# Orkis-Research/Quaternion-Convolutional-Neural-Networks-for-End-to-End-Automatic-Speech-Recognition

Measured on AMD Instinct MI355X. Metric: quaternion-conv samples/sec (fwd+bwd+Adam of the full TIMIT QCNN, per-GPU batch 256), higher is better.
Workload: dtype bf16; 1 GPU; cfg3_qcnn_relu_dropout_b256_bf16; per_gpu_batch=256, global_batch=256, filters=32, padding=same, activation=relu, loss=ctc, parallelism=dp1, optimizer=adam(5e-4) + l2 term folded into the update, launch=eager

## Files before the change

### quaternion-convolutional-neural-networks-for-end-to-end-automatic-speech-recognition_amd/csrc/qk_common.h

```cpp
#pragma once

#include <hip/hip_runtime.h>
#include <stdint.h>
#include <stdio.h>
#include <stdlib.h>

#include "../../include/qk.h"

namespace qk {

constexpr unsigned kSignConv = 0x5390u;
constexpr unsigned kSignConj = 0x284Eu;

struct PostOp {
    int kind;
    int alpha_sel;
    int alpha_len;
    const float *alpha;
    float drop_scale;
    unsigned drop_thr;
    unsigned drop_seed;
    const unsigned *seed_dev;
};

struct GemmGeom {
    int M;
    int batch;
    int osp[3];
    int isp[3];
    int Q;
    int J;
    int Qp, Jp;
    int ks[3];
    int taps;
    int pa[3], pb[3], pc[3], pd[3];
    long long in_sn, in_ss[3], in_sc;
    long long out_sn, out_ss, out_sc;
    unsigned sign_tbl;
    int relu;
    int has_bias;
    int has_mask;
    int ablate;
    unsigned b_rep;
    unsigned long long *dbg_ts;
    int w_swapped;
    int w_prepped;
    unsigned dv_mul[3], dv_shr[3];
    const void *ep_mask;
    PostOp post;
    int post_fwd;
    void *pre_out;
    float *dalpha;
    void *bits_out;
    const void *ep_bits;
    int b_wp, b_nlines, b_cshift, b_rev;
    int o0_major;
    unsigned b_in_bytes, b_w_bytes;
    int w_ch_major;
};

inline int pad32(int v) { return (v + 31) / 32 * 32; }
inline size_t band_image_bytes(int taps, int Qp, int Jp) { return (size_t)taps * Qp * 4 * Jp * 2 + 256; }

inline bool band_geom(const GemmGeom &g, int esize, GemmGeom *o)
{
    if (g.has_mask) return false;
    if (g.pd[0] != 1 || g.pd[1] != 1 || g.pd[2] != 1) return false;
    int ax = 2;
    while (ax > 0 && g.osp[ax] == 1 && g.isp[ax] == 1 && g.ks[ax] == 1) --ax;
    if (g.ks[ax] != 3 && g.ks[ax] != 5) return false;
    if (g.pa[ax] != 1 || (g.pb[ax] != 1 && g.pb[ax] != -1)) return false;
    *o = g;
    const int sh = 2 - ax;
    for (int i = 0; i < 3; ++i) {
        const int src = i - sh;
        o->osp[i] = src >= 0 ? g.osp[src] : 1; o->isp[i] = src >= 0 ? g.isp[src] : 1; o->ks[i] = src >= 0 ? g.ks[src] : 1;
        o->pa[i] = src >= 0 ? g.pa[src] : 1; o->pb[i] = src >= 0 ? g.pb[src] : 1; o->pc[i] = src >= 0 ? g.pc[src] : 0;
        o->in_ss[i] = src >= 0 ? g.in_ss[src] : 0;
    }
    const int k = o->ks[2];
    if (o->ks[0] * o->ks[1] > 32) return false;
    for (int i = 0; i < 2; ++i)
        if (o->pb[i] != 1 && o->pb[i] != -1) return false;
    o->b_rep = 0;
    for (int t0 = 0; t0 < o->ks[0]; ++t0) o->b_rep |= 1u << (t0 * o->ks[1]);
    o->b_wp = o->osp[2] + k - 1;
    if ((k - 1) * 12 > o->b_wp) return false;
    const long long lines = (long long)g.batch * o->osp[0] * o->osp[1];
    if (lines * o->b_wp >= (1ll << 31) - 512) return false;
    o->b_nlines = (int)lines;
    const int Qw = g.Qp ? g.Qp : g.Q, Jw = g.Jp ? g.Jp : g.J;
    const long long in_bytes = (long long)g.batch * g.in_sn * esize, w_bytes = (long long)band_image_bytes(g.taps, Qw, Jw);
    if (in_bytes >= 0xF0000000ll || w_bytes >= 0xF0000000ll) return false;
    o->b_in_bytes = (unsigned)in_bytes;
    o->b_w_bytes = (unsigned)w_bytes;
    o->b_rev = o->pb[2] < 0;
    o->b_cshift = o->b_rev ? o->pc[2] - (k - 1) : o->pc[2];
    if (o->post.alpha_sel >= 0) o->post.alpha_sel += sh;
    return true;
}


inline void fastdiv_of(unsigned d, unsigned *mul, unsigned *shr)
{
    if (d <= 1) { *mul = 0; *shr = 0; return; }
    unsigned lg = 0;
    while ((1ull << lg) < d) ++lg;
    const unsigned p = 31 + lg;
    *mul = (unsigned)(((1ull << p) + d - 1) / d);
    *shr = p - 32;
}
__device__ __forceinline__ int fastdiv(int n, unsigned mul, unsigned shr)
{
    const unsigned q = __umulhi((unsigned)n, mul) >> shr;
    const unsigned id = (unsigned)-(int)(mul == 0u);
    return (int)((q & ~id) | ((unsigned)n & id));
}

__device__ __forceinline__ unsigned outer_tap_mask(int q0, int q1, const GemmGeom &g)
{
    const int m0 = q0 * g.pb[0] + (g.pb[0] > 0 ? 0 : g.isp[0] - 1), m1q = q1 * g.pb[1] + (g.pb[1] > 0 ? 0 : g.isp[1] - 1);
    const int lo0 = max(0, -m0), hi0 = min(g.ks[0], g.isp[0] - m0);
    const int lo1 = max(0, -m1q), hi1 = min(g.ks[1], g.isp[1] - m1q);
    const unsigned m1 = ((hi1 >= 32 ? 0u : (1u << hi1)) - 1u) & ~((1u << lo1) - 1u);
    const int b0 = lo0 * g.ks[1], e0 = hi0 * g.ks[1];
    const unsigned r0 = ((e0 >= 32 ? 0u : (1u << e0)) - 1u) & ~((1u << b0) - 1u);
    return (lo0 >= hi0 || lo1 >= hi1) ? 0u : (m1 * g.b_rep) & r0;
}


struct WgradGeom {
    int M;
    int batch;
    int osp[3];
    int isp[3];
    int Cq, F;
    int ks[3];
    int taps;
    int pa[3], pb[3], pc[3];
    long long x_sn, x_ss[3], x_sc;
    long long dy_sn, dy_ss, dy_sc;
    unsigned sign_tbl;
    int has_mask;
    int want_dbias;
    int m_per_split;
    int n_splits;
    int ablate;
    int deterministic;
    unsigned x_bytes, dy_bytes;
    int b_wp, b_nlines, b_cshift;
    int w_ch_major;
    void *dym;
    unsigned fd_mul[4], fd_sh[4];
};

inline void make_fastdiv(unsigned d, unsigned *mul, unsigned *sh)
{
    unsigned s = 0;
    while ((1ull << s) < d) ++s;
    *mul = (unsigned)(((1ull << (31 + s)) + d - 1) / d);
    *sh = s;
}
__host__ __device__ __forceinline__ int fast_div(int n, unsigned mul, unsigned sh)
{
    return (int)(((unsigned long long)(unsigned)n * mul) >> (31 + sh));
}

struct bf16 { uint16_t x; };
typedef _Float16 f16;

__device__ __forceinline__ float to_f32(float v) { return v; }
__device__ __forceinline__ float to_f32(bf16 v) { return __uint_as_float(((uint32_t)v.x) << 16); }
__device__ __forceinline__ float to_f32(f16 v) { return (float)v; }

template <typename T> __device__ __forceinline__ T from_f32(float v);
template <> __device__ __forceinline__ float from_f32<float>(float v) { return v; }
template <> __device__ __forceinline__ bf16 from_f32<bf16>(float v)
{
    uint32_t u = __float_as_uint(v);
    bf16 r;
    if ((u & 0x7fffffffu) > 0x7f800000u) { r.x = (uint16_t)((u >> 16) | 0x40u); return r; }
    u += 0x7fffu + ((u >> 16) & 1u);
    r.x = (uint16_t)(u >> 16);
    return r;
}
template <> __device__ __forceinline__ f16 from_f32<f16>(float v) { return (f16)v; }

__device__ __forceinline__ void load4(const float *p, float (&o)[4])
{
    const float4 v = *reinterpret_cast<const float4 *>(p);
    o[0] = v.x; o[1] = v.y; o[2] = v.z; o[3] = v.w;
}
__device__ __forceinline__ void load4(const bf16 *p, float (&o)[4])
{
    const uint2 v = *reinterpret_cast<const uint2 *>(p);
    o[0] = __uint_as_float(v.x << 16); o[1] = __uint_as_float(v.x & 0xffff0000u);
    o[2] = __uint_as_float(v.y << 16); o[3] = __uint_as_float(v.y & 0xffff0000u);
}
__device__ __forceinline__ void load4(const f16 *p, float (&o)[4])
{
    typedef f16 h4 __attribute__((ext_vector_type(4)));
    const h4 v = *reinterpret_cast<const h4 *>(p);
    o[0] = (float)v[0]; o[1] = (float)v[1]; o[2] = (float)v[2]; o[3] = (float)v[3];
}

template <typename T>
__device__ __forceinline__ void prep_small16_write(const float *w, T *wq, long long idx, int Cq, int F, int transposed, int neg_ijk,
// ... 142 lines not shown
```

### quaternion-convolutional-neural-networks-for-end-to-end-automatic-speech-recognition_amd/csrc/qk_hgemm_bf16mfma.hip

```cpp
#include "qk_common.h"
#include "qk_postop.h"
#include <type_traits>

namespace qk {
namespace {

typedef __bf16 bf16x8 __attribute__((ext_vector_type(8)));
typedef _Float16 f16x8 __attribute__((ext_vector_type(8)));

__device__ __forceinline__ floatx16 mfma16(bf16, const uint4 &a, const uint4 &b, const floatx16 &c)
{
    return __builtin_amdgcn_mfma_f32_32x32x16_bf16(__builtin_bit_cast(bf16x8, a), __builtin_bit_cast(bf16x8, b), c, 0, 0, 0);
}
__device__ __forceinline__ floatx16 mfma16(f16, const uint4 &a, const uint4 &b, const floatx16 &c)
{
    return __builtin_amdgcn_mfma_f32_32x32x16_f16(__builtin_bit_cast(f16x8, a), __builtin_bit_cast(f16x8, b), c, 0, 0, 0);
}

typedef float f32x2 __attribute__((ext_vector_type(2)));
typedef __bf16 bf16x2 __attribute__((ext_vector_type(2)));
typedef _Float16 f16x2 __attribute__((ext_vector_type(2)));
__device__ __forceinline__ unsigned pack2(bf16, float a, float b)
{
    const f32x2 v = {a, b};
// ... 1083 lines not shown

inline bool point_geom(const GemmGeom &g, GemmGeom *o)
{
    if (g.has_mask || (g.Q != 32 && g.Q != 64) || g.J % 32 != 0) return false;
    if (g.post.kind != 0) {
        const bool epm = g.ep_mask || g.ep_bits;
        const bool fwd_relu = g.post_fwd && g.post.kind == 2 && !g.pre_out && !epm;
        if (!fwd_relu && (!epm || g.post_fwd || g.post.alpha_len > 256 || (g.taps == 1 && g.post.alpha_sel >= 0))) return false;
    }
    *o = g;
    if (g.taps == 1) {
        for (int i = 0; i < 3; ++i)
            if (g.pa[i] != 1 || g.pc[i] != 0 || g.isp[i] != g.osp[i]) return false;
        if (g.in_ss[1] != g.isp[2] * g.in_ss[2] || g.in_ss[0] != g.isp[1] * g.in_ss[1] || g.in_sn != g.isp[0] * g.in_ss[0]) return false;
        o->batch = g.M;
        o->in_sn = g.in_ss[2];
        for (int i = 0; i < 3; ++i) { o->osp[i] = o->isp[i] = 1; o->in_ss[i] = 0; }
    } else {
        if (g.ks[1] != 1 || g.ks[2] != 1 || g.isp[0] != 1 || g.ks[0] != g.osp[0]) return false;
        for (int i = 1; i < 3; ++i)
            if (g.pa[i] != 1 || g.pc[i] != 0 || g.isp[i] != g.osp[i]) return false;
        if (g.pc[0] != 0 || g.pa[0] != 1 || g.pb[0] != -1) return false;
    }
    if ((long long)o->batch * o->in_sn * 2 >= (1ll << 31) || (long long)g.M * g.out_ss >= (1ll << 31)) return false;
    return true;
}

template <typename T>
int run16_point(const T *in, const uint4 *wq, const float *bias, T *out, GemmGeom g, hipStream_t stream)
{
    const int S = g.osp[1] * g.osp[2], R = g.batch * S;
    fastdiv_of((unsigned)g.osp[2], &g.dv_mul[0], &g.dv_shr[0]);
    fastdiv_of((unsigned)g.osp[1], &g.dv_mul[1], &g.dv_shr[1]);
    fastdiv_of((unsigned)S, &g.dv_mul[2], &g.dv_shr[2]);
    const bool wide = g.J % 64 == 0;
    const int BM = wide ? 128 : 256, BF = wide ? 64 : 32;
    const int n_tiles = (R + BM - 1) / BM;
    const int n_units = g.ks[0] * (g.J / BF) * n_tiles;
    int blocks = device_cu_count();
    if (blocks > n_units) blocks = n_units;
    const unsigned in_bytes = (unsigned)((long long)g.batch * g.in_sn * 2);
    const unsigned out_bytes = (unsigned)((long long)g.M * g.out_ss * 2);
#define QK_GO(NKC, E, W) hipLaunchKernelGGL((k_hgemm16_point<T, NKC, E, W>), dim3(blocks), dim3(512), 0, stream, in, wq, bias, out, g, n_tiles, n_units, in_bytes, out_bytes)
    const int epm = g.ep_bits ? 2 : g.ep_mask ? 1 : 0;
#define QK_GO3(NKC, W) do { if (epm == 2) QK_GO(NKC, 2, W); else if (epm == 1) QK_GO(NKC, 1, W); else QK_GO(NKC, 0, W); } while (0)
    if (wide) { if (g.Q == 64) QK_GO3(2, 2); else QK_GO3(1, 2); }
    else      { if (g.Q == 64) QK_GO3(2, 1); else QK_GO3(1, 1); }
#undef QK_GO3
#undef QK_GO
    return hipGetLastError() == hipSuccess ? 1 : QK_ERR_LAUNCH;
}

template <typename T, int WM, int WN, int KIN, bool TRIM, bool PAD = false>
int run16_band(const T *in, const uint4 *wq, const T *zero_line, const float *bias, T *out, const GemmGeom &g,
               hipStream_t stream)
{
    constexpr int BM = WM * 32, BF = WN * 32, BMU = TRIM ? BM - (KIN - 1) : BM, NTHR = WM * WN * 64;
    const int n_mt = (int)(((long long)g.b_nlines * g.b_wp + BMU - 1) / BMU);
    dim3 grid((n_mt + 7) / 8 * 8, (PAD ? g.Jp : g.J) / BF, 1);
#define QK_GO(C, E, P) hipLaunchKernelGGL((k_hgemm16_band<T, WM, WN, KIN, C, TRIM, E, P, PAD>), grid, dim3(NTHR), (g.ablate & 64) ? 40960 : 0, stream, in, wq, zero_line, bias, out, g)
    const bool epm = g.ep_mask != nullptr, pf = g.post.kind != 0 && g.post_fwd != 0;
    if (g.sign_tbl != kSignConj) return QK_ERR_LAUNCH;
    if constexpr (!PAD && WM * WN == 4) {
        if (g.ep_bits) { QK_GO(true, 2, false); return hipGetLastError() == hipSuccess ? 1 : QK_ERR_LAUNCH; }
    }
    if (g.ep_bits || ((PAD || WM * WN != 4) && g.bits_out)) return QK_ERR_UNSUPPORTED;
    if (epm) QK_GO(true, 1, false); else if (pf) QK_GO(true, 0, true); else QK_GO(true, 0, false);
#undef QK_GO
    return hipGetLastError() == hipSuccess ? 1 : QK_ERR_LAUNCH;
}

template <typename T, int MT, int WM, int WN>
int run16(const T *in, const T *mask, const uint4 *wq, const T *zero_line, const float *bias, T *out,
          const GemmGeom &g_in, hipStream_t stream)
{
    constexpr int BM = WM * MT * 32, BF = WN * 32;
    const GemmGeom &g = g_in;
    const int n_mt = (g.M + BM - 1) / BM;
    dim3 grid((n_mt + 7) / 8 * 8, g.J / BF, 1);
    const bool m = g.has_mask != 0;
    if (g.sign_tbl != kSignConj) return QK_ERR_LAUNCH;
#define QK_GO(C, K) hipLaunchKernelGGL((k_hgemm16<T, MT, WM, WN, C, K>), grid, dim3(512), 0, stream, in, mask, wq, zero_line, bias, out, g)
    if (m) QK_GO(true, true); else QK_GO(true, false);
#undef QK_GO
    return hipGetLastError() == hipSuccess ? 1 : QK_ERR_LAUNCH;
}

template <typename T>
int go16(const void *in, const void *mask, const float *w, const float *bias, void *out, const GemmGeom &g_in,
         bool transposed, void *ws, size_t ws_bytes, hipStream_t stream)
{
    GemmGeom g = g_in;
    g.ablate = debug_ablate();
    { size_t nb = 0; g.dbg_ts = debug_buffer(&nb); if (nb < 64u * 65536u) g.dbg_ts = nullptr; }
    const bool neg_ijk = g.sign_tbl == kSignConv;
    g.sign_tbl = kSignConj;
    for (int i = 0; i < 3; ++i) fastdiv_of((unsigned)g.osp[2 - i], &g.dv_mul[i], &g.dv_shr[i]);
    T *wq = static_cast<T *>(ws);
    const int Cq = transposed ? g.J : g.Q, F = transposed ? g.Q : g.J;
    g.Qp = pad32(g.Q); g.Jp = pad32(g.J);
    const bool padded = g.Qp != g.Q || g.Jp != g.J;
    const bool bits = g.bits_out || g.ep_bits;
    if (bits && (padded || g.post.kind != 2)) return QK_ERR_UNSUPPORTED;
    GemmGeom bg;
    {
        Small16 sm;
        const size_t band_bytes = band_image_bytes(g.taps, g.Qp, g.Jp);
        if (!g.w_ch_major && small16_shape(g, &bg, &sm) && ws_bytes >= band_bytes + small16_region_bytes(sm)) {
            T *wqs = reinterpret_cast<T *>(static_cast<char *>(ws) + band_bytes);
            if (!g.w_prepped) {
// ... 127 lines not shown
```

### quaternion-convolutional-neural-networks-for-end-to-end-automatic-speech-recognition_amd/csrc/qk_hgemm_f32mfma.inc

```

namespace qk {
namespace {

struct RowPos { int n, o0, o1, o2; };

__device__ __forceinline__ RowPos decompose(int m, int M, const int (&osp)[3])
{
    RowPos r;
    if (m >= M) { r.n = -1; r.o0 = r.o1 = r.o2 = 0; return r; }
    int s = m;
    r.o2 = s % osp[2]; s /= osp[2];
    r.o1 = s % osp[1]; s /= osp[1];
    r.o0 = s % osp[0];
    r.n = s / osp[0];
    return r;
}

__device__ __forceinline__ bool axis_pos(int o, int t, int pa, int pb, int pc, int pd, int isp, int &i)
{
    const int num = o * pa + t * pb + pc;
    i = num;
    bool ok = num >= 0;
    if (pd != 1) {
        i = num / pd;
// ... 696 lines not shown
                    } else {
                        const int P = pt0 + row;
                        line = P / WP;
                        u = P - line * WP;
                    }
                    if (line >= g.b_nlines || u >= g.osp[2] || nvalid <= 0) continue;
                    float *dst = reinterpret_cast<float *>(out) + (size_t)(line * g.osp[2] + u) * (size_t)g.out_ss + ech;
                    if (nvalid >= 4) {
                        *reinterpret_cast<float4 *>(dst) = v;
                    } else {
                        dst[0] = v.x;
                        if (nvalid > 1) dst[1] = v.y;
                        if (nvalid > 2) dst[2] = v.z;
                    }
                }
            }
            return;
        }
    }
#pragma unroll
    for (int t = 0; t < NTILE; ++t) {
        if (!TP::valid(wave, t)) continue;
        const int jslot = TP::b_slot(t);
        const int j = j0 + cj[jslot];
        if (j >= g.J) continue;
        const int ch = cb[jslot] * g.J + j;
        const float bia = g.has_bias ? bias[ch] : 0.f;
        const int pt0 = p0 + TP::a_tile(wave, TP::a_slot(t)) * 32;
#pragma unroll
        for (int r = 0; r < 16; ++r) {
            int line, u;
            if (two_lines) {
                const int rr = rem0 + (pt0 - p0) + mfma32_row(r, lane);
                const bool second = rr >= WP;
                line = line0 + (second ? 1 : 0);
                u = second ? rr - WP : rr;
            } else {
                const int P = pt0 + mfma32_row(r, lane);
                line = P / WP;
                u = P - line * WP;
            }
            if (line >= g.b_nlines || u >= g.osp[2]) continue;
            float v = ((WIDE && w_sigma) ? -acc[t][r] : acc[t][r]) + bia;
            if (g.relu) v = v > 0.f ? v : 0.f;
            out[(line * g.osp[2] + u) * (int)g.out_ss + ch] = from_f32<T>(v);
        }
    }
}

template <typename T, typename TP, int BQ, int KIN>
int run_hgemm_band(const T *in, const float *wk, const float *bias, T *out, const GemmGeom &g, hipStream_t stream)
{
    constexpr int BM = TP::BMT * 32, BJ = TP::BNT * 8;
    const long long n_mt = ((long long)g.b_nlines * g.b_wp + BM - 1) / BM;
    const long long n_tiles = n_mt * ((g.J + BJ - 1) / BJ);
    dim3 grid((unsigned)((n_tiles + 7) / 8 * 8), 1, 1);
    GemmGeom ga = g;
    ga.ablate = debug_ablate();
    hipLaunchKernelGGL((k_hgemm_band<T, TP, BQ, KIN>), grid, dim3(TP::NW * 64), 0, stream, in, wk, bias, out, ga);
    return hipGetLastError() == hipSuccess ? 0 : QK_ERR_LAUNCH;
}

template <typename T, int RT, int CT, int NW, int BKM, bool VEC, bool MASK>
__global__ void __launch_bounds__(NW * 64)
k_wgrad(const T *__restrict__ x, const T *__restrict__ dy, const T *__restrict__ ymask,
        float *__restrict__ dw, float *__restrict__ dbias, const WgradGeom g)
{
    constexpr int BC = RT * 8;
    constexpr int BF = NW * CT * 8;
    constexpr int NTHR = NW * 64;
    constexpr int BCP = BC + (BC % 16 == 0 ? 8 : 0);
    constexpr int BFP = BF + (BF % 16 == 0 ? 8 : 0);
    constexpr int XS = 4 * BCP + (VEC ? 0 : 1);
    constexpr int DS = 4 * BFP + (VEC ? 0 : 1);
    constexpr int MAIN = BKM * (XS + DS);
    constexpr int FOLD = BC * 4 * BF;
    constexpr bool DB = 2 * MAIN * 4 <= 128 * 1024;
    constexpr int LDSF = (DB ? 2 : 1) * MAIN > FOLD ? (DB ? 2 : 1) * MAIN : FOLD;
    __shared__ __attribute__((aligned(16))) float lds[LDSF];
    float *Xs = lds;
    float *Dsm = lds + BKM * XS;

    const int tid = threadIdx.x;
    const int lane = tid & 63;
    const int wave = __builtin_amdgcn_readfirstlane(tid >> 6);
    const int lr = lane & 31, lk = lane >> 5;
    const int nfc = (g.F + BF - 1) / BF;
    const int cchunk = blockIdx.y / nfc;
    const int fchunk = blockIdx.y - cchunk * nfc;
    const int c0 = cchunk * BC, f0 = fchunk * BF;
    const int t = blockIdx.z;
    const int t2 = t % g.ks[2];
    const int tt = t / g.ks[2];
    const int t1 = tt % g.ks[1];
    const int t0 = tt / g.ks[1];
    const int m_begin = blockIdx.x * g.m_per_split;
    const int m_end = min(g.M, m_begin + g.m_per_split);
    const int S = g.osp[0] * g.osp[1] * g.osp[2];
    const bool do_bias = g.want_dbias && t == 0 && cchunk == 0;

    constexpr int TPR = NTHR / BKM;
    constexpr int UX = (BC + TPR - 1) / TPR;
    constexpr int UD = BF / TPR;
    constexpr int GX = 4 * BC / TPR;
    constexpr int GD = 4 * BF / TPR;
    static_assert(BF % TPR == 0 && (4 * BC) % TPR == 0, "tile/threads");
    float xr[VEC ? UX : 1][4];
    float dr[VEC ? UD : 1][4];
    float mr[(VEC && MASK) ? UD : 1][4];
    float xg[VEC ? 1 : GX];
// ... 296 lines not shown
                   const GemmGeom &g, bool vec, hipStream_t stream)
{
    typedef TilesProduct<1, 2, 2, 4> P0;
    typedef TilesProduct<2, 2, 2, 4> P1;
    typedef TilesProduct<1, 1, 4, 1> P2;
    typedef TilesProduct<1, 1, 4, 2> P3;
    typedef TilesProduct<1, 2, 4, 2> P4;
    typedef TilesFlat<2, 5, 8> F5;
    typedef TilesFlat<4, 5, 8> F6;
    static const HgemmCfg cands[] = {
        {0, 2, 8, 8, 8}, {0, 2, 8, 8, 16}, {0, 2, 8, 8, 32}, {0, 2, 8, 8, 40},
        {1, 4, 8, 8, 8}, {1, 4, 8, 8, 16}, {1, 4, 8, 8, 32},
        {2, 4, 1, 4, 8}, {2, 4, 1, 4, 16}, {2, 4, 1, 4, 32},
        {3, 4, 2, 8, 8}, {3, 4, 2, 8, 32},
        {4, 4, 4, 8, 8}, {4, 4, 4, 8, 32},
        {5, 2, 5, 8, 8}, {5, 2, 5, 8, 32}, {5, 2, 5, 8, 40},
        {6, 4, 5, 8, 8}, {6, 4, 5, 8, 16}, {6, 4, 5, 8, 32},
    };
    int best = -1;
    double best_cost = 0;
    for (int i = 0; i < (int)(sizeof(cands) / sizeof(cands[0])); ++i) {
        const HgemmCfg &c = cands[i];
        if (!vec && c.bq != 8) continue;
        const int BM = c.bmt * 32, BJ = c.bnt * 8;
        const long long blocks = (((long long)g.M + BM - 1) / BM) * ((g.J + BJ - 1) / BJ);
        const long long nq = (g.Q + c.bq - 1) / c.bq;
        const int tile_steps = (c.bmt * c.bnt + 3) / 4;
        const long long tile_bytes = 4LL * (4 * c.bq * (BM + 1) + c.bq * 4 * BJ);
        const long long lds_bytes = (2 * tile_bytes <= 160 * 1024) ? 2 * tile_bytes : tile_bytes;
        long long occ = 160 * 1024 / lds_bytes;
        if (occ > 32 / c.nw) occ = 32 / c.nw;
        if (occ < 1) occ = 1;
        const double mfma = (double)g.taps * nq * tile_steps * 4.0 * (c.bq / 2) * 64.0 * 1.3;
        const double ovh = (double)g.taps * nq * 2500.0 + tile_steps * 1500.0 + 6000.0;
        const double cost = (double)((blocks + 255) / 256) * mfma + (double)((blocks + 256 * occ - 1) / (256 * occ)) * ovh;
        if (best < 0 || cost < best_cost) { best = i; best_cost = cost; }
    }
    if (vec && g.taps <= 5 && g.M >= 8192 && g.M <= 16384) {
        const int want_id = (g.Q == 40 && g.J == 64) ? 0 : (g.Q == 64 && g.J == 40) ? 2 : -1;
        const int want_bq = want_id == 0 ? 40 : 16;
        for (int i = 0; want_id >= 0 && i < (int)(sizeof(cands) / sizeof(cands[0])); ++i)
            if (cands[i].id == want_id && cands[i].bq == want_bq) best = i;
    }
    int force_id = -1, force_bq = -1;
    const bool forced = debug_force_cfg(&force_id, &force_bq);
    if (forced)
        for (int i = 0; i < (int)(sizeof(cands) / sizeof(cands[0])); ++i)
            if (cands[i].id == force_id && cands[i].bq == force_bq && (vec || force_bq == 8)) best = i;
    if constexpr (sizeof(T) == 4) {
        GemmGeom bg;
        const long long S_out = (long long)g.osp[0] * g.osp[1] * g.osp[2];
        if (vec && !(debug_flags() & kDbgNoBand32) && !forced && g.out_sn == S_out * g.out_ss && band_geom(g, 4, &bg)) {
            const bool k3 = bg.ks[2] == 3;
            const long long big_tiles = (((long long)bg.b_nlines * bg.b_wp + 127) / 128) * ((g.J + 63) / 64);
            if (big_tiles >= 1024 && g.Q % 8 == 0) {
                if (g.Q % 32 == 0)
                    return k3 ? run_hgemm_band<T, P1, 32, 3>(in, wk, bias, out, bg, stream)
                              : run_hgemm_band<T, P1, 32, 5>(in, wk, bias, out, bg, stream);
                if (g.Q % 16 == 0)
                    return k3 ? run_hgemm_band<T, P1, 16, 3>(in, wk, bias, out, bg, stream)
                              : run_hgemm_band<T, P1, 16, 5>(in, wk, bias, out, bg, stream);
                return k3 ? run_hgemm_band<T, P1, 8, 3>(in, wk, bias, out, bg, stream)
                          : run_hgemm_band<T, P1, 8, 5>(in, wk, bias, out, bg, stream);
            }
            if (cands[best].id == 0 && cands[best].bq == 40 && g.Q % 8 == 0)
                return k3 ? run_hgemm_band<T, P0, 40, 3>(in, wk, bias, out, bg, stream)
                          : run_hgemm_band<T, P0, 40, 5>(in, wk, bias, out, bg, stream);
            if (cands[best].id == 2 && g.Q % 16 == 0)
                return k3 ? run_hgemm_band<T, P2, 16, 3>(in, wk, bias, out, bg, stream)
                          : run_hgemm_band<T, P2, 16, 5>(in, wk, bias, out, bg, stream);
        }
    }
    const HgemmCfg &c = cands[best];
#define QK_CASE(ID, TP, BQ_) \
    if (c.id == ID && c.bq == BQ_) return run_hgemm<T, TP, BQ_>(in, mask, wk, bias, out, g, vec, stream);
    QK_CASE(0, P0, 8) QK_CASE(0, P0, 16) QK_CASE(0, P0, 32) QK_CASE(0, P0, 40)
    QK_CASE(1, P1, 8) QK_CASE(1, P1, 16) QK_CASE(1, P1, 32)
    QK_CASE(2, P2, 8) QK_CASE(2, P2, 16) QK_CASE(2, P2, 32)
    QK_CASE(3, P3, 8) QK_CASE(3, P3, 32)
    QK_CASE(4, P4, 8) QK_CASE(4, P4, 32)
    QK_CASE(5, F5, 8) QK_CASE(5, F5, 32) QK_CASE(5, F5, 40)
    QK_CASE(6, F6, 8) QK_CASE(6, F6, 16) QK_CASE(6, F6, 32)
#undef QK_CASE
    return QK_ERR_UNSUPPORTED;
}

template <typename T, int RT, int CT, int NW, int BKM>
int run_wgrad(const T *x, const T *dy, const T *ymask, float *dw, float *dbias, WgradGeom g,
              bool vec, hipStream_t stream)
{
    constexpr int BC = RT * 8, BF = NW * CT * 8;
    const int ncc = (g.Cq + BC - 1) / BC, nfc = (g.F + BF - 1) / BF;
    const long long other = (long long)ncc * nfc * g.taps;
    const long long max_splits = ((long long)g.M + BKM - 1) / BKM;
    const long long n_cu = 256, kEpilogueSteps = 3;
    long long splits = 1, best_cost = -1;
    for (int r = 1; r <= 3; ++r) {
        long long sp = r * n_cu / other;
        sp = sp < 1 ? 1 : (sp > max_splits ? max_splits : sp);
        long long mps_r = (g.M + sp - 1) / sp;
        mps_r = (mps_r + BKM - 1) / BKM * BKM;
        sp = (g.M + mps_r - 1) / mps_r;
        const long long per_cu = (sp * other + n_cu - 1) / n_cu;
        const long long cost = per_cu * (mps_r / BKM + kEpilogueSteps);
        if (best_cost < 0 || cost < best_cost) { best_cost = cost; splits = sp; }
    }
    g.deterministic = (debug_flags() & kDbgDeterministic) ? 1 : 0;
// ... 59 lines not shown
```

### quaternion-convolutional-neural-networks-for-end-to-end-automatic-speech-recognition_amd/csrc/qk_wgrad_band_bf16mfma.hip

```cpp
#include "qk_common.h"

namespace qk {
namespace {

typedef __bf16 bf16x8 __attribute__((ext_vector_type(8)));
typedef _Float16 f16x8 __attribute__((ext_vector_type(8)));
typedef short v4s __attribute__((ext_vector_type(4)));
typedef short v8s __attribute__((ext_vector_type(8)));

__device__ __forceinline__ floatx16 mfma16b(bf16, const v8s &a, const v8s &b, const floatx16 &c)
{
    return __builtin_amdgcn_mfma_f32_32x32x16_bf16(__builtin_bit_cast(bf16x8, a), __builtin_bit_cast(bf16x8, b), c, 0, 0, 0);
}
__device__ __forceinline__ floatx16 mfma16b(f16, const v8s &a, const v8s &b, const floatx16 &c)
{
    return __builtin_amdgcn_mfma_f32_32x32x16_f16(__builtin_bit_cast(f16x8, a), __builtin_bit_cast(f16x8, b), c, 0, 0, 0);
}

typedef __attribute__((address_space(3))) v4s lds_v4s;
__device__ __forceinline__ v8s tr_frag8(const char *base, int pitch)
{
    const v4s lo = __builtin_amdgcn_ds_read_tr16_b64_v4i16((lds_v4s *)(base));
    const v4s hi = __builtin_amdgcn_ds_read_tr16_b64_v4i16((lds_v4s *)(base + 4 * pitch));
    return __builtin_shufflevector(lo, hi, 0, 1, 2, 3, 4, 5, 6, 7);
}

typedef unsigned int u32x4 __attribute__((ext_vector_type(4)));
constexpr unsigned kOOR = 0xF0000000u;
__device__ __forceinline__ __amdgpu_buffer_rsrc_t rsrc_of(const void *p, unsigned bytes)
{
    return __builtin_amdgcn_make_buffer_rsrc(const_cast<void *>(p), 0, (int)bytes, 0x00020000);
}
__device__ __forceinline__ uint4 bload16(__amdgpu_buffer_rsrc_t r, unsigned voff, unsigned soff)
{
    const u32x4 v = __builtin_amdgcn_raw_buffer_load_b128(r, (int)voff, (int)soff, 0);
    return make_uint4(v.x, v.y, v.z, v.w);
}
__device__ __forceinline__ void bstore16(const uint4 &d, __amdgpu_buffer_rsrc_t r, unsigned voff, unsigned soff)
{
    u32x4 v; v.x = d.x; v.y = d.y; v.z = d.z; v.w = d.w;
    __builtin_amdgcn_raw_buffer_store_b128(v, r, (int)(voff + soff), 0, 0);
}
typedef unsigned short u2v __attribute__((ext_vector_type(2)));
__device__ __forceinline__ unsigned keep2(unsigned v, unsigned m)
{
    const u2v one = __builtin_elementwise_min(__builtin_bit_cast(u2v, m), (u2v)(1));
    return v & __builtin_bit_cast(unsigned, (u2v)(one * (u2v)(0xffff)));
}

template <typename T, int RTT, int KIN, bool MASK, int CTW>
__global__ void __launch_bounds__(512) __attribute__((amdgpu_waves_per_eu(2, 2)))
k_wgrad16_band(const T *__restrict__ x, const T *__restrict__ dy, const T *__restrict__ ymask,
               float *__restrict__ dw, float *__restrict__ dbias, const WgradGeom g)
{
    static_assert(RTT == 2 || RTT == 4, "row tiles per tap");
    static_assert(KIN == 3 || KIN == 5, "inner taps");
    static_assert(CTW == 1 || CTW == 2, "column tiles per wave");
    constexpr int NTHR = 512, WCG = 8 / RTT;
    constexpr int CQB = RTT * 8, BF = WCG * CTW * 8;
    constexpr int KM = 64;
    constexpr int XROW = 4 * CQB * 2 + 64, DROW = 4 * BF * 2 + 64;
    constexpr int XBUF = (KM + KIN - 1) * XROW, DBUF = KM * DROW, BUF = XBUF + DBUF;
    constexpr int FOLD = KIN * CQB * 4 * BF * 4;
    static_assert(2 * BUF >= FOLD, "fold slab reuses the tile buffers");
    __shared__ __attribute__((aligned(16))) char lds[2 * BUF];

    const int tid = threadIdx.x;
    const int lane = tid & 63;
    const int wave = __builtin_amdgcn_readfirstlane(tid >> 6);
    const int rt = wave / WCG, cg = wave % WCG;
    const int n_ot = g.ks[0] * g.ks[1];
    const int ncc = g.Cq / CQB, nfc = g.F / BF;
    const int n_inner = n_ot * ncc * nfc;
    const int n_tiles = n_inner * g.n_splits;
    const int per_xcd = (n_tiles + 7) / 8;
    const int tile = (blockIdx.x % 8) * per_xcd + blockIdx.x / 8;
    if (tile >= n_tiles) return;
    const int split = tile / n_inner;
    const int inner = tile - split * n_inner;
    const int ot = inner % n_ot;
    const int chunk = inner / n_ot;
    const int cchunk = chunk / nfc, fchunk = chunk - cchunk * nfc;
    const int c0 = cchunk * CQB, f0 = fchunk * BF;
    const int t0 = ot / g.ks[1], t1 = ot - t0 * g.ks[1];
    const int WP = g.b_wp, W = g.osp[2];
    const int p_begin = split * g.m_per_split;
    const int p_end = min(g.b_nlines * WP, p_begin + g.m_per_split);
    const bool share0 = ot * ncc + cchunk == 0;
    const int n_share = g.deterministic ? (share0 ? 1 : (1 << 30)) : n_ot * ncc;
    const bool bias_blk = g.want_dbias != 0, dym_blk = MASK && g.dym != nullptr;
    int turn = g.deterministic ? (share0 ? 0 : (1 << 29)) : ot * ncc + cchunk;

    constexpr int UC = CQB / 8, UF = BF / 8;
    constexpr int UX = (4 * UC) / 8, UD = (4 * UF) / 8;
    static_assert(UX >= 1 && UD >= 1, "units per thread");
    const int s_row = tid >> 3, s_sub = tid & 7;
    const __amdgpu_buffer_rsrc_t rx = rsrc_of(x, g.x_bytes), rdy = rsrc_of(dy, g.dy_bytes);
    const __amdgpu_buffer_rsrc_t ry = rsrc_of(MASK ? ymask : dy, g.dy_bytes);
    const __amdgpu_buffer_rsrc_t rdym = rsrc_of(g.dym ? g.dym : dy, g.dym ? g.dy_bytes : 0u);
    const unsigned x_thr = (unsigned)((s_sub / UC) * g.Cq + c0 + (s_sub % UC) * 8) * 2u;
    const unsigned d_thr = (unsigned)((s_sub / UF) * g.F + f0 + (s_sub % UF) * 8) * 2u;
    const unsigned x_ustep = (unsigned)((8 / UC) * g.Cq) * 2u, d_ustep = (unsigned)((8 / UF) * g.F) * 2u;
    uint4 xr[UX], xh[UX], dr[UD], mr[MASK ? UD : 1];
    int r_line, r_u, r_o0, r_o1, r_i0, r_i1;
    unsigned xo2, dyo2;
    const int W_ = g.osp[2];
    {
        const int P = p_begin + s_row;
        r_line = P / WP; r_u = P - r_line * WP;
        int l = r_line;
        r_o1 = l % g.osp[1]; l /= g.osp[1];
        r_o0 = l % g.osp[0];
        const int r_n = l / g.osp[0];
// ... 199 lines not shown
                        float *dst = &slab[((t * CQB + cc) * 4 + p) * BF + ff];
                        *dst = ph == 0 ? v : *dst + v;
                    }
                }
            }
        }
        __syncthreads();
    }
    const int tap0 = ot * KIN;
    for (int e = tid; e < KIN * CQB * 4 * BF; e += NTHR) {
        const int ff = e % BF;
        const int p = (e / BF) & 3;
        const int cv = e / (4 * BF);
        const int t = cv / CQB, cc = cv - t * CQB;
        if (!(g.ablate & 2))
            atomicAdd(dw + (((tap0 + t) * g.Cq + c0 + cc) * 4 + p) * g.F + f0 + ff, slab[e]);
    }
    if (bias_blk && tid < 4 * BF) {
        const int b = tid / BF, ff = tid % BF;
        atomicAdd(dbias + b * g.F + f0 + ff, dbacc);
    }
}


typedef __attribute__((address_space(3))) char lds_char;
typedef __attribute__((address_space(3))) void lds_void_t;
typedef __bf16 bf16x2_t __attribute__((ext_vector_type(2)));
typedef _Float16 f16x2_t __attribute__((ext_vector_type(2)));
__device__ __forceinline__ float dot_ones(bf16, unsigned w, float c)
{
    return __builtin_amdgcn_fdot2_f32_bf16(__builtin_bit_cast(bf16x2_t, w), __builtin_bit_cast(bf16x2_t, 0x3F803F80u), c, false);
}
__device__ __forceinline__ float dot_ones(f16, unsigned w, float c)
{
    return __builtin_amdgcn_fdot2(__builtin_bit_cast(f16x2_t, w), __builtin_bit_cast(f16x2_t, 0x3C003C00u), c, false);
}
__device__ __forceinline__ v8s tr_pair(const lds_char *p)
{
    const v4s lo = __builtin_amdgcn_ds_read_tr16_b64_v4i16((lds_v4s *)(p));
    const v4s hi = __builtin_amdgcn_ds_read_tr16_b64_v4i16((lds_v4s *)(p + 512));
    return __builtin_shufflevector(lo, hi, 0, 1, 2, 3, 4, 5, 6, 7);
}

template <typename T, int RTT, int KIN, bool PAD = false, int CTW = 2>
__global__ void __launch_bounds__(512) __attribute__((amdgpu_waves_per_eu(2, 2)))
k_wgrad16_band3(const T *__restrict__ x, const T *__restrict__ dy, float *__restrict__ dw, float *__restrict__ dbias, const WgradGeom g)
{
    static_assert(!PAD || RTT == 4 || CTW == 1, "padded channel counts: the 32 x 32 block form, or 16 x 32 with an exact channel side");
    static_assert(CTW == 2 || (CTW == 1 && RTT == 2), "column tiles per wave");
    static_assert(RTT == 2 || RTT == 4, "row tiles per tap");
    static_assert(KIN == 3 || KIN == 5, "inner taps");
    constexpr int NTHR = 512, WCG = 8 / RTT;
    constexpr int CQB = RTT * 8, BF = WCG * CTW * 8;
    constexpr int KM = 64, KS = KM / 16, NMF = KIN * CTW;
    constexpr int NPX = (4 * CQB * 2) / 128, NPD = (4 * BF * 2) / 128;
    constexpr int XROWS = KM + 8;
    constexpr int XPL = XROWS * 128, DPL = KM * 128;
    constexpr int DOFF = NPX * XPL;
    constexpr int BUFB = NPX * XPL + NPD * DPL;
    constexpr int TAPB = CQB * 4 * BF * 4;
    static_assert(2 * TAPB <= BUFB, "two taps of the fold slab per tile buffer");
    static_assert((KIN + 1) / 2 <= 3, "three tile buffers");
    __shared__ __attribute__((aligned(1024))) char lds0[BUFB];
    __shared__ __attribute__((aligned(1024))) char lds1[BUFB];
    __shared__ __attribute__((aligned(1024))) char lds2[BUFB];

    const int tid = threadIdx.x;
    const int lane = tid & 63;
    const int wave = __builtin_amdgcn_readfirstlane(tid >> 6);
    const int rt = wave / WCG, cg = wave % WCG;
    const int n_ot = g.ks[0] * g.ks[1];
    const int ncc = (g.Cq + CQB - 1) / CQB, nfc = (g.F + BF - 1) / BF;
    const int n_inner = n_ot * ncc * nfc;
    const int n_tiles = n_inner * g.n_splits;
    const int per_xcd = (n_tiles + 7) / 8;
    const int tile = (blockIdx.x % 8) * per_xcd + blockIdx.x / 8;
    if (tile >= n_tiles) return;
    const int split = tile / n_inner;
    const int inner = tile - split * n_inner;
    const int ot = inner % n_ot;
    const int chunk = inner / n_ot;
    const int cchunk = chunk / nfc, fchunk = chunk - cchunk * nfc;
    const int c0 = cchunk * CQB, f0 = fchunk * BF;
    const int t0 = ot / g.ks[1], t1 = ot - t0 * g.ks[1];
    const int WP = g.b_wp, W = g.osp[2];
    const int p_begin = split * g.m_per_split;
    const int p_end = min(g.b_nlines * WP, p_begin + g.m_per_split);
    const bool share0 = ot * ncc + cchunk == 0;
    const int n_share = g.deterministic ? (share0 ? 1 : (1 << 30)) : n_ot * ncc;
    const bool bias_wave = g.want_dbias != 0 && rt == 0;
    int turn = g.deterministic ? (share0 ? 0 : (1 << 29)) : ot * ncc + cchunk;

    constexpr int UC = CQB / 8, UF = BF / 8;
    const int s_row = tid >> 3, s_sub = tid & 7;
    const int s_src = s_sub ^ (((s_row >> 1) & 1) << 2);
    const __amdgpu_buffer_rsrc_t rx = rsrc_of(x, g.x_bytes), rdy = rsrc_of(dy, g.dy_bytes);
    const unsigned x_thr = (unsigned)((s_src / UC) * g.Cq + c0 + (s_src % UC) * 8) * 2u;
    const unsigned d_thr = (unsigned)((s_src / UF) * g.F + f0 + (s_src % UF) * 8) * 2u;
    const unsigned x_pstep = (unsigned)((8 / UC) * g.Cq) * 2u, d_pstep = (unsigned)((8 / UF) * g.F) * 2u;
    const bool x_grp_ok = !PAD || c0 + (s_src % UC) * 8 < g.Cq, d_grp_ok = !PAD || f0 + (s_src % UF) * 8 < g.F;
    const unsigned xs2 = (unsigned)((int)g.x_ss[2]) * 2u, dys = (unsigned)((int)g.dy_ss) * 2u;
    int su0, Pj, lineB, nB, o0B, o1B;
    unsigned xbA, xbB, dbA, dbB;
    int xvA, xvB, dvA, dvB;
    auto line_vals = [&](int line, int n, int o0, int o1, unsigned &xb, int &xv, unsigned &db, int &dv) {
        const int i0 = o0 * g.pa[0] + t0 * g.pb[0] + g.pc[0], i1 = o1 * g.pa[1] + t1 * g.pb[1] + g.pc[1];
        dv = line < g.b_nlines;
// ... 159 lines not shown
    const int lr = lane & 31;
#pragma unroll
    for (int ph = 0; ph < 4; ++ph) {
        const bool active = RTT == 2 ? rt == (ph >> 1) : rt == ph;
        if (active) {
#pragma unroll
            for (int ct = 0; ct < CTW; ++ct) {
                const int col = (cg * CTW + ct) * 32 + lr;
                const int b = col / BF, ff = col % BF;
                const int p = ph ^ b;
                const bool neg = (g.sign_tbl >> (ph * 4 + b)) & 1u;
#pragma unroll
                for (int r = 0; r < 16; ++r) {
                    if (RTT == 2 && (r >> 3) != (ph & 1)) continue;
                    const int row = mfma32_row(r, lane);
                    const int cc = RTT == 2 ? (row & 15) : row;
#pragma unroll
                    for (int t = 0; t < KIN; ++t) {
                        float *slab = reinterpret_cast<float *>(t / 2 == 0 ? lds0 : t / 2 == 1 ? lds1 : lds2) + (t & 1) * (TAPB / 4);
                        const float v = neg ? -acc[t][ct][r] : acc[t][ct][r];
                        float *dst = &slab[(cc * 4 + p) * BF + ff];
                        *dst = ph == 0 ? v : *dst + v;
                    }
                }
            }
        }
        __syncthreads();
    }
    const int tap0 = ot * KIN;
#pragma unroll
    for (int t = 0; t < KIN; ++t) {
        const float *slab = reinterpret_cast<const float *>(t / 2 == 0 ? lds0 : t / 2 == 1 ? lds1 : lds2) + (t & 1) * (TAPB / 4);
        for (int e = tid; e < CQB * 4 * BF; e += NTHR) {
            const int ff = e % BF;
            const int p = (e / BF) & 3;
            const int cc = e / (4 * BF);
            if (!(g.ablate & 2) && (!PAD || (c0 + cc < g.Cq && f0 + ff < g.F)))
                atomicAdd(dw + (((tap0 + t) * g.Cq + c0 + cc) * 4 + p) * g.F + f0 + ff, slab[e]);
        }
    }
    if (bias_wave) {
#pragma unroll
        for (int ct = 0; ct < CTW; ++ct) {
            const float s = dbacc[ct] + __shfl_xor(dbacc[ct], 32);
            const int col = (cg * CTW + ct) * 32 + lr;
            if (lane < 32 && (!PAD || f0 + col % BF < g.F)) atomicAdd(dbias + (col / BF) * g.F + f0 + col % BF, s);
        }
    }
}

template <typename T, int RTT, int KIN, int CTW = 2, bool LINEAR_NARROW = false>
int run_wgrad16_band(const T *x, const T *dy, const T *ymask, float *dw, float *dbias, WgradGeom g, hipStream_t stream)
{
    constexpr int CQB = RTT * 8, BF = (8 / RTT) * CTW * 8, KM = 64;
    const bool padded = g.Cq % CQB != 0 || g.F % BF != 0;
    const long long other = (long long)g.ks[0] * g.ks[1] * ((g.Cq + CQB - 1) / CQB) * ((g.F + BF - 1) / BF);
    const long long total_p = (long long)g.b_nlines * g.b_wp;
    const long long max_splits = (total_p + KM - 1) / KM;
    const int slots = device_cu_count();
    const long long kEpilogueSteps = 24;
    long long splits = 1, best_cost = -1;
    for (int r = 1; r <= 4; ++r) {
        long long sp = (long long)r * slots / other;
        sp = sp < 1 ? 1 : (sp > max_splits ? max_splits : sp);
        long long mps_r = (total_p + sp - 1) / sp;
        mps_r = (mps_r + KM - 1) / KM * KM;
        sp = (total_p + mps_r - 1) / mps_r;
        const long long rounds = (sp * other + slots - 1) / slots;
        const long long cost = rounds * (mps_r / KM + kEpilogueSteps);
        if (best_cost < 0 || cost < best_cost) { best_cost = cost; splits = sp; }
    }
    g.deterministic = (debug_flags() & kDbgDeterministic) ? 1 : 0;
    if (g.deterministic) splits = 1;
    long long mps = (total_p + splits - 1) / splits;
    mps = (mps + KM - 1) / KM * KM;
    splits = (total_p + mps - 1) / mps;
    g.m_per_split = (int)mps;
    g.n_splits = (int)splits;
    g.x_bytes = (unsigned)((long long)g.batch * g.x_sn * 2);
    g.dy_bytes = (unsigned)((long long)g.M * g.dy_ss * 2);
    g.ablate = debug_ablate();
    const long long n_tiles = splits * other;
    dim3 grid((unsigned)((n_tiles + 7) / 8 * 8), 1, 1);
    constexpr bool kMasked = !(RTT == 2 && KIN == 5 && CTW == 2) && !LINEAR_NARROW, kLinear = !(RTT == 2 && KIN == 5 && CTW == 1) && !LINEAR_NARROW;
    constexpr bool kNarrow = RTT == 2 && CTW == 1 && LINEAR_NARROW;
    if (padded || kNarrow) {
        if constexpr ((RTT == 4 && CTW == 2) || kNarrow) {
            if (g.has_mask || g.dym || g.b_wp < KM + 8) return 0;
            if (padded) hipLaunchKernelGGL((k_wgrad16_band3<T, RTT, KIN, true, CTW>), grid, dim3(512), 0, stream, x, dy, dw, dbias, g);
            else hipLaunchKernelGGL((k_wgrad16_band3<T, RTT, KIN, false, CTW>), grid, dim3(512), 0, stream, x, dy, dw, dbias, g);
        } else return 0;
    } else if (g.has_mask) {
        if constexpr (kMasked) hipLaunchKernelGGL((k_wgrad16_band<T, RTT, KIN, true, CTW>), grid, dim3(512), 0, stream, x, dy, ymask, dw, dbias, g);
        else return QK_ERR_UNSUPPORTED;
    } else if (CTW == 2 && !g.dym && g.b_wp >= KM + 8 && !(debug_flags() & kDbgWgradBandV1)) {
        if constexpr (CTW == 2) hipLaunchKernelGGL((k_wgrad16_band3<T, RTT, KIN>), grid, dim3(512), 0, stream, x, dy, dw, dbias, g);
    } else {
        if constexpr (kLinear) hipLaunchKernelGGL((k_wgrad16_band<T, RTT, KIN, false, CTW>), grid, dim3(512), 0, stream, x, dy, ymask, dw, dbias, g);
        else return QK_ERR_UNSUPPORTED;
    }
    return hipGetLastError() == hipSuccess ? 1 : QK_ERR_LAUNCH;
}

bool wgrad_band_geom(const WgradGeom &g, WgradGeom *o)
{
    int ax = 2;
    while (ax > 0 && g.osp[ax] == 1 && g.isp[ax] == 1 && g.ks[ax] == 1) --ax;
    if (g.ks[ax] != 3 && g.ks[ax] != 5) return false;
    if (g.pa[ax] != 1 || g.pb[ax] != 1) return false;
    *o = g;
    const int sh = 2 - ax;
    for (int i = 0; i < 3; ++i) {
        const int src = i - sh;
        o->osp[i] = src >= 0 ? g.osp[src] : 1; o->isp[i] = src >= 0 ? g.isp[src] : 1; o->ks[i] = src >= 0 ? g.ks[src] : 1;
        o->pa[i] = src >= 0 ? g.pa[src] : 1; o->pb[i] = src >= 0 ? g.pb[src] : 1; o->pc[i] = src >= 0 ? g.pc[src] : 0;
        o->x_ss[i] = src >= 0 ? g.x_ss[src] : 0;
    }
    const int k = o->ks[2];
    o->b_wp = o->osp[2] + k - 1;
    if ((k - 1) * 12 > o->b_wp) return false;
    const long long lines = (long long)g.batch * o->osp[0] * o->osp[1];
    if (lines * o->b_wp >= (1ll << 31) - 512) return false;
    o->b_nlines = (int)lines;
    o->b_cshift = o->pc[2];
    return true;
}

template <typename T>
int go_wgrad16_band(const void *x, const void *dy, const void *ymask, float *dw, float *dbias, const WgradGeom &g,
                    hipStream_t stream)
{
    const T *xp = (const T *)x, *dp = (const T *)dy, *yp = (const T *)ymask;
    const bool k5 = g.ks[2] == 5;
    if (g.F % 64 == 0 && g.Cq % 16 == 0 && !(g.has_mask && g.Cq % 32 == 0)) {
        if (g.has_mask && k5) return run_wgrad16_band<T, 2, 5, 1>(xp, dp, yp, dw, dbias, g, stream);
        return k5 ? run_wgrad16_band<T, 2, 5>(xp, dp, yp, dw, dbias, g, stream) : run_wgrad16_band<T, 2, 3>(xp, dp, yp, dw, dbias, g, stream);
    }
    if (g.Cq % 32 != 0 && !g.has_mask)
        return k5 ? run_wgrad16_band<T, 2, 5, 1, true>(xp, dp, yp, dw, dbias, g, stream) : run_wgrad16_band<T, 2, 3, 1, true>(xp, dp, yp, dw, dbias, g, stream);
    return k5 ? run_wgrad16_band<T, 4, 5>(xp, dp, yp, dw, dbias, g, stream) : run_wgrad16_band<T, 4, 3>(xp, dp, yp, dw, dbias, g, stream);
}

}

int try_wgrad_band_16(int dtype, const void *x, const void *dy, const void *ymask, float *dw, float *dbias,
                      const WgradGeom &g, hipStream_t stream)
{
    if (dtype != QK_BF16 && dtype != QK_F16) return 0;
    if (debug_flags() & (kDbgNoMfma16 | kDbgNoWgradBand)) return 0;
    if (g.x_sc != 1 || g.dy_sc != 1) return 0;
    const long long S = (long long)g.osp[0] * g.osp[1] * g.osp[2];
    if (g.dy_sn != S * g.dy_ss) return 0;
    if (g.F % 16 != 0 || g.Cq % 16 != 0) return 0;
    if (g.has_mask && (g.F % 32 != 0 || g.Cq % (g.F % 64 == 0 ? 16 : 32) != 0)) return 0;
    if ((long long)g.batch * g.x_sn * 2 >= 0xF0000000ll || (long long)g.M * g.dy_ss * 2 >= 0xF0000000ll) return 0;
    if ((reinterpret_cast<uintptr_t>(x) | reinterpret_cast<uintptr_t>(dy) | reinterpret_cast<uintptr_t>(ymask)) & 15) return 0;
    WgradGeom bg;
    if (!wgrad_band_geom(g, &bg)) return 0;
    if ((long long)bg.taps * bg.Cq * 4 * bg.F >= (1ll << 31)) return 0;
    note_path(QK_PATH_MFMA16_BAND);
    if (dtype == QK_BF16) return go_wgrad16_band<bf16>(x, dy, ymask, dw, dbias, bg, stream);
    return go_wgrad16_band<f16>(x, dy, ymask, dw, dbias, bg, stream);
}

}
```

Before: 14890 samples/s.

## Shrink band line pitch to cut padded rows in band conv and wgrad

Band kernels linearize each line with pitch out+k-1. This change computes a tighter pitch from the actual leading and trailing zero padding, bounded below by the output width and by the tile-row floors each kernel needs. Fewer padded positions means fewer M tiles and wgrad K-steps. The wgrad split-cost model now also accounts for the band3 kernel stepping in groups of three. This risks correctness if any kernel assumed the full padded pitch.

```diff
diff --git a/quaternion-convolutional-neural-networks-for-end-to-end-automatic-speech-recognition_amd/csrc/qk_common.h b/quaternion-convolutional-neural-networks-for-end-to-end-automatic-speech-recognition_amd/csrc/qk_common.h
--- a/quaternion-convolutional-neural-networks-for-end-to-end-automatic-speech-recognition_amd/csrc/qk_common.h
+++ b/quaternion-convolutional-neural-networks-for-end-to-end-automatic-speech-recognition_amd/csrc/qk_common.h
@@ -62,6 +62,24 @@
 inline int pad32(int v) { return (v + 31) / 32 * 32; }
 inline size_t band_image_bytes(int taps, int Qp, int Jp) { return (size_t)taps * Qp * 4 * Jp * 2 + 256; }
 
+inline int band_line_pitch(int in, int out, int k, int cshift, int floor0 = 0, int floor1 = 0)
+{
+    const int full = out + k - 1;
+    const int lead = -cshift, trail = full - lead - in;
+    int zeros = lead > trail ? lead : trail;
+    if (zeros < 0) zeros = 0;
+    int pitch = in + zeros;
+    if (pitch < out) pitch = out;
+    if (pitch > full) pitch = full;
+    if ((pitch < floor0 && full >= floor0) || (pitch < floor1 && full >= floor1)) pitch = full;
+    return pitch;
+}
+inline bool band_lines_admitted(int out, int k, long long lines)
+{
+    if ((k - 1) * 12 > out + k - 1) return false;
+    return lines * (out + k - 1) < (1ll << 31) - 512;
+}
+
 inline bool band_geom(const GemmGeom &g, int esize, GemmGeom *o)
 {
     if (g.has_mask) return false;
@@ -84,10 +102,8 @@
         if (o->pb[i] != 1 && o->pb[i] != -1) return false;
     o->b_rep = 0;
     for (int t0 = 0; t0 < o->ks[0]; ++t0) o->b_rep |= 1u << (t0 * o->ks[1]);
-    o->b_wp = o->osp[2] + k - 1;
-    if ((k - 1) * 12 > o->b_wp) return false;
     const long long lines = (long long)g.batch * o->osp[0] * o->osp[1];
-    if (lines * o->b_wp >= (1ll << 31) - 512) return false;
+    if (!band_lines_admitted(o->osp[2], k, lines)) return false;
     o->b_nlines = (int)lines;
     const int Qw = g.Qp ? g.Qp : g.Q, Jw = g.Jp ? g.Jp : g.J;
     const long long in_bytes = (long long)g.batch * g.in_sn * esize, w_bytes = (long long)band_image_bytes(g.taps, Qw, Jw);
@@ -96,6 +112,7 @@
     o->b_w_bytes = (unsigned)w_bytes;
     o->b_rev = o->pb[2] < 0;
     o->b_cshift = o->b_rev ? o->pc[2] - (k - 1) : o->pc[2];
+    o->b_wp = band_line_pitch(o->isp[2], o->osp[2], k, o->b_cshift);
     if (o->post.alpha_sel >= 0) o->post.alpha_sel += sh;
     return true;
 }
@@ -109,6 +126,11 @@
     const unsigned p = 31 + lg;
     *mul = (unsigned)(((1ull << p) + d - 1) / d);
     *shr = p - 32;
+}
+inline void band_pitch_floor(GemmGeom *g, int band_rows)
+{
+    g->b_wp = band_line_pitch(g->isp[2], g->osp[2], g->ks[2], g->b_cshift, band_rows);
+    fastdiv_of((unsigned)g->b_wp, &g->dv_mul[0], &g->dv_shr[0]);
 }
 __device__ __forceinline__ int fastdiv(int n, unsigned mul, unsigned shr)
 {
@@ -153,6 +175,30 @@
     void *dym;
     unsigned fd_mul[4], fd_sh[4];
 };
+
+constexpr int kWgradBandKM = 64;
+inline bool wgrad_band_geom(const WgradGeom &g, WgradGeom *o)
+{
+    int ax = 2;
+    while (ax > 0 && g.osp[ax] == 1 && g.isp[ax] == 1 && g.ks[ax] == 1) --ax;
+    if (g.ks[ax] != 3 && g.ks[ax] != 5) return false;
+    if (g.pa[ax] != 1 || g.pb[ax] != 1) return false;
+    *o = g;
+    const int sh = 2 - ax;
+    for (int i = 0; i < 3; ++i) {
+        const int src = i - sh;
+        o->osp[i] = src >= 0 ? g.osp[src] : 1; o->isp[i] = src >= 0 ? g.isp[src] : 1; o->ks[i] = src >= 0 ? g.ks[src] : 1;
+        o->pa[i] = src >= 0 ? g.pa[src] : 1; o->pb[i] = src >= 0 ? g.pb[src] : 1; o->pc[i] = src >= 0 ? g.pc[src] : 0;
+        o->x_ss[i] = src >= 0 ? g.x_ss[src] : 0;
+    }
+    const int k = o->ks[2];
+    const long long lines = (long long)g.batch * o->osp[0] * o->osp[1];
+    if (!band_lines_admitted(o->osp[2], k, lines)) return false;
+    o->b_nlines = (int)lines;
+    o->b_cshift = o->pc[2];
+    o->b_wp = band_line_pitch(o->isp[2], o->osp[2], k, o->b_cshift, kWgradBandKM + 8, kWgradBandKM);
+    return true;
+}
 
 inline void make_fastdiv(unsigned d, unsigned *mul, unsigned *sh)
 {
diff --git a/quaternion-convolutional-neural-networks-for-end-to-end-automatic-speech-recognition_amd/csrc/qk_hgemm_bf16mfma.hip b/quaternion-convolutional-neural-networks-for-end-to-end-automatic-speech-recognition_amd/csrc/qk_hgemm_bf16mfma.hip
--- a/quaternion-convolutional-neural-networks-for-end-to-end-automatic-speech-recognition_amd/csrc/qk_hgemm_bf16mfma.hip
+++ b/quaternion-convolutional-neural-networks-for-end-to-end-automatic-speech-recognition_amd/csrc/qk_hgemm_bf16mfma.hip
@@ -1159,10 +1159,12 @@
 }
 
 template <typename T, int WM, int WN, int KIN, bool TRIM, bool PAD = false>
-int run16_band(const T *in, const uint4 *wq, const T *zero_line, const float *bias, T *out, const GemmGeom &g,
+int run16_band(const T *in, const uint4 *wq, const T *zero_line, const float *bias, T *out, const GemmGeom &g_in,
                hipStream_t stream)
 {
     constexpr int BM = WM * 32, BF = WN * 32, BMU = TRIM ? BM - (KIN - 1) : BM, NTHR = WM * WN * 64;
+    GemmGeom g = g_in;
+    band_pitch_floor(&g, TRIM ? BM : BM + KIN - 1);
     const int n_mt = (int)(((long long)g.b_nlines * g.b_wp + BMU - 1) / BMU);
     dim3 grid((n_mt + 7) / 8 * 8, (PAD ? g.Jp : g.J) / BF, 1);
 #define QK_GO(C, E, P) hipLaunchKernelGGL((k_hgemm16_band<T, WM, WN, KIN, C, TRIM, E, P, PAD>), grid, dim3(NTHR), (g.ablate & 64) ? 40960 : 0, stream, in, wq, zero_line, bias, out, g)
diff --git a/quaternion-convolutional-neural-networks-for-end-to-end-automatic-speech-recognition_amd/csrc/qk_hgemm_f32mfma.inc b/quaternion-convolutional-neural-networks-for-end-to-end-automatic-speech-recognition_amd/csrc/qk_hgemm_f32mfma.inc
--- a/quaternion-convolutional-neural-networks-for-end-to-end-automatic-speech-recognition_amd/csrc/qk_hgemm_f32mfma.inc
+++ b/quaternion-convolutional-neural-networks-for-end-to-end-automatic-speech-recognition_amd/csrc/qk_hgemm_f32mfma.inc
@@ -772,10 +772,11 @@
 int run_hgemm_band(const T *in, const float *wk, const float *bias, T *out, const GemmGeom &g, hipStream_t stream)
 {
     constexpr int BM = TP::BMT * 32, BJ = TP::BNT * 8;
-    const long long n_mt = ((long long)g.b_nlines * g.b_wp + BM - 1) / BM;
+    GemmGeom ga = g;
+    band_pitch_floor(&ga, BM + KIN - 1);
+    const long long n_mt = ((long long)ga.b_nlines * ga.b_wp + BM - 1) / BM;
     const long long n_tiles = n_mt * ((g.J + BJ - 1) / BJ);
     dim3 grid((unsigned)((n_tiles + 7) / 8 * 8), 1, 1);
-    GemmGeom ga = g;
     ga.ablate = debug_ablate();
     hipLaunchKernelGGL((k_hgemm_band<T, TP, BQ, KIN>), grid, dim3(TP::NW * 64), 0, stream, in, wk, bias, out, ga);
     return hipGetLastError() == hipSuccess ? 0 : QK_ERR_LAUNCH;
@@ -1178,7 +1179,7 @@
         const long long S_out = (long long)g.osp[0] * g.osp[1] * g.osp[2];
         if (vec && !(debug_flags() & kDbgNoBand32) && !forced && g.out_sn == S_out * g.out_ss && band_geom(g, 4, &bg)) {
             const bool k3 = bg.ks[2] == 3;
-            const long long big_tiles = (((long long)bg.b_nlines * bg.b_wp + 127) / 128) * ((g.J + 63) / 64);
+            const long long big_tiles = (((long long)bg.b_nlines * (bg.osp[2] + bg.ks[2] - 1) + 127) / 128) * ((g.J + 63) / 64);
             if (big_tiles >= 1024 && g.Q % 8 == 0) {
                 if (g.Q % 32 == 0)
                     return k3 ? run_hgemm_band<T, P1, 32, 3>(in, wk, bias, out, bg, stream)
diff --git a/quaternion-convolutional-neural-networks-for-end-to-end-automatic-speech-recognition_amd/csrc/qk_wgrad_band_bf16mfma.hip b/quaternion-convolutional-neural-networks-for-end-to-end-automatic-speech-recognition_amd/csrc/qk_wgrad_band_bf16mfma.hip
--- a/quaternion-convolutional-neural-networks-for-end-to-end-automatic-speech-recognition_amd/csrc/qk_wgrad_band_bf16mfma.hip
+++ b/quaternion-convolutional-neural-networks-for-end-to-end-automatic-speech-recognition_amd/csrc/qk_wgrad_band_bf16mfma.hip
@@ -58,7 +58,7 @@
     static_assert(CTW == 1 || CTW == 2, "column tiles per wave");
     constexpr int NTHR = 512, WCG = 8 / RTT;
     constexpr int CQB = RTT * 8, BF = WCG * CTW * 8;
-    constexpr int KM = 64;
+    constexpr int KM = kWgradBandKM;
     constexpr int XROW = 4 * CQB * 2 + 64, DROW = 4 * BF * 2 + 64;
     constexpr int XBUF = (KM + KIN - 1) * XROW, DBUF = KM * DROW, BUF = XBUF + DBUF;
     constexpr int FOLD = KIN * CQB * 4 * BF * 4;
@@ -364,7 +364,7 @@
     static_assert(KIN == 3 || KIN == 5, "inner taps");
     constexpr int NTHR = 512, WCG = 8 / RTT;
     constexpr int CQB = RTT * 8, BF = WCG * CTW * 8;
-    constexpr int KM = 64, KS = KM / 16, NMF = KIN * CTW;
+    constexpr int KM = kWgradBandKM, KS = KM / 16, NMF = KIN * CTW;
     constexpr int NPX = (4 * CQB * 2) / 128, NPD = (4 * BF * 2) / 128;
     constexpr int XROWS = KM + 8;
     constexpr int XPL = XROWS * 128, DPL = KM * 128;
@@ -630,13 +630,16 @@
 template <typename T, int RTT, int KIN, int CTW = 2, bool LINEAR_NARROW = false>
 int run_wgrad16_band(const T *x, const T *dy, const T *ymask, float *dw, float *dbias, WgradGeom g, hipStream_t stream)
 {
-    constexpr int CQB = RTT * 8, BF = (8 / RTT) * CTW * 8, KM = 64;
+    constexpr int CQB = RTT * 8, BF = (8 / RTT) * CTW * 8, KM = kWgradBandKM;
+    constexpr bool kNarrow = RTT == 2 && CTW == 1 && LINEAR_NARROW;
     const bool padded = g.Cq % CQB != 0 || g.F % BF != 0;
     const long long other = (long long)g.ks[0] * g.ks[1] * ((g.Cq + CQB - 1) / CQB) * ((g.F + BF - 1) / BF);
     const long long total_p = (long long)g.b_nlines * g.b_wp;
     const long long max_splits = (total_p + KM - 1) / KM;
     const int slots = device_cu_count();
     const long long kEpilogueSteps = 24;
+    const bool band3 = padded || kNarrow || (!g.has_mask && CTW == 2 && !g.dym && g.b_wp >= KM + 8 && !(debug_flags() & kDbgWgradBandV1));
+    auto steps_run = [&](long long iters) { return band3 ? (iters + 1) / 3 * 3 + 1 : iters; };
     long long splits = 1, best_cost = -1;
     for (int r = 1; r <= 4; ++r) {
         long long sp = (long long)r * slots / other;
@@ -645,7 +648,7 @@
         mps_r = (mps_r + KM - 1) / KM * KM;
         sp = (total_p + mps_r - 1) / mps_r;
         const long long rounds = (sp * other + slots - 1) / slots;
-        const long long cost = rounds * (mps_r / KM + kEpilogueSteps);
+        const long long cost = rounds * (steps_run(mps_r / KM) + kEpilogueSteps);
         if (best_cost < 0 || cost < best_cost) { best_cost = cost; splits = sp; }
     }
     g.deterministic = (debug_flags() & kDbgDeterministic) ? 1 : 0;
@@ -661,7 +664,6 @@
     const long long n_tiles = splits * other;
     dim3 grid((unsigned)((n_tiles + 7) / 8 * 8), 1, 1);
     constexpr bool kMasked = !(RTT == 2 && KIN == 5 && CTW == 2) && !LINEAR_NARROW, kLinear = !(RTT == 2 && KIN == 5 && CTW == 1) && !LINEAR_NARROW;
-    constexpr bool kNarrow = RTT == 2 && CTW == 1 && LINEAR_NARROW;
     if (padded || kNarrow) {
         if constexpr ((RTT == 4 && CTW == 2) || kNarrow) {
             if (g.has_mask || g.dym || g.b_wp < KM + 8) return 0;
@@ -671,37 +673,13 @@
     } else if (g.has_mask) {
         if constexpr (kMasked) hipLaunchKernelGGL((k_wgrad16_band<T, RTT, KIN, true, CTW>), grid, dim3(512), 0, stream, x, dy, ymask, dw, dbias, g);
         else return QK_ERR_UNSUPPORTED;
-    } else if (CTW == 2 && !g.dym && g.b_wp >= KM + 8 && !(debug_flags() & kDbgWgradBandV1)) {
+    } else if (band3) {
         if constexpr (CTW == 2) hipLaunchKernelGGL((k_wgrad16_band3<T, RTT, KIN>), grid, dim3(512), 0, stream, x, dy, dw, dbias, g);
     } else {
         if constexpr (kLinear) hipLaunchKernelGGL((k_wgrad16_band<T, RTT, KIN, false, CTW>), grid, dim3(512), 0, stream, x, dy, ymask, dw, dbias, g);
         else return QK_ERR_UNSUPPORTED;
     }
     return hipGetLastError() == hipSuccess ? 1 : QK_ERR_LAUNCH;
-}
-
-bool wgrad_band_geom(const WgradGeom &g, WgradGeom *o)
-{
-    int ax = 2;
-    while (ax > 0 && g.osp[ax] == 1 && g.isp[ax] == 1 && g.ks[ax] == 1) --ax;
-    if (g.ks[ax] != 3 && g.ks[ax] != 5) return false;
-    if (g.pa[ax] != 1 || g.pb[ax] != 1) return false;
-    *o = g;
-    const int sh = 2 - ax;
-    for (int i = 0; i < 3; ++i) {
-        const int src = i - sh;
-        o->osp[i] = src >= 0 ? g.osp[src] : 1; o->isp[i] = src >= 0 ? g.isp[src] : 1; o->ks[i] = src >= 0 ? g.ks[src] : 1;
-        o->pa[i] = src >= 0 ? g.pa[src] : 1; o->pb[i] = src >= 0 ? g.pb[src] : 1; o->pc[i] = src >= 0 ? g.pc[src] : 0;
-        o->x_ss[i] = src >= 0 ? g.x_ss[src] : 0;
-    }
-    const int k = o->ks[2];
-    o->b_wp = o->osp[2] + k - 1;
-    if ((k - 1) * 12 > o->b_wp) return false;
-    const long long lines = (long long)g.batch * o->osp[0] * o->osp[1];
-    if (lines * o->b_wp >= (1ll << 31) - 512) return false;
-    o->b_nlines = (int)lines;
-    o->b_cshift = o->pc[2];
-    return true;
 }
 
 template <typename T>
```

Result: no change. 14970 samples/s, median of 6 (+0.5%).
